# gevaertlab/sequoia-pub

Hardware: AMD Instinct MI355X
Metric: slides/sec (1000-patch WSI, UNI-dim, 20k-gene head) (higher is better)
Workload: dtype f16x3; 1 GPU; pipeline: 1000 x 224x224 uint8 patches/slide -> ResNet-50 embed -> k-Means(100) -> ViS(D=2048, depth 6, 16 heads, G=20820) forward (BASELINE config 3), patches uploaded from pinned host memory every step; embedder=ResNet-50 (src/resnet.py forward_extract), feature_dim=2048, patch_size=224, parallelism=slide-sharded x1

## Files before the change

### sequoia-pub_amd/csrc/conv1_x3.hip

```cpp
#include "gemm.h"
#include "x3_fmt.h"

namespace {

constexpr int TP = 8;
constexpr int TC = 2 * TP + 1;
constexpr int RW = 40;
constexpr int RH = 2 * TC + 5;
constexpr int IN_BYTES = RH * RW * 8;
constexpr int MT = 10;
constexpr int CROW = 272;
constexpr int COUT_BYTES = MT * 32 * CROW;
constexpr int LUT_BYTES = 2 * 3 * 256 * 2;
constexpr int W_LD = 152;
constexpr int NT = 512;
constexpr int RW_BYTES = 16384;
constexpr int LDS_BYTES = 2 * IN_BYTES + COUT_BYTES + LUT_BYTES + RW_BYTES;

struct Conv1X3Args {
    const uint8_t* u8;
    const float* f32;
    const uint16_t* w;
    long long w_plane;
    const float* bias;
    const float* colscale;
    uint16_t* out;
    long long out_plane;
    int n, H, W, tiles_y, tiles_x, tiles;
    const uint16_t* w1;
    int w1_tiled;
    const float* b1; const float* cs1;
    uint16_t* t1;
};

template <bool F16>
__global__ __launch_bounds__(NT) void conv1_pool_x3_kernel(const Conv1X3Args p) {
    using F = X3Fmt<F16>;
    extern __shared__ __attribute__((aligned(16))) char smem[];
    char* s_hi = smem;
    char* s_lo = smem + IN_BYTES;
    char* s_out = smem + 2 * IN_BYTES;
    uint16_t* s_lut = reinterpret_cast<uint16_t*>(smem + 2 * IN_BYTES + COUT_BYTES);
    const int tid = threadIdx.x, lane = tid & 63;
    const int wave = __builtin_amdgcn_readfirstlane(tid >> 6);
    const int wm = wave >> 1, wn = wave & 1;
    const int l31 = lane & 31, g = lane >> 5;
    const int tile0 = wm < 2 ? wm * 3 : 6 + (wm - 2) * 2;
    const int ntile = wm < 2 ? 3 : 2;

    for (int i = tid; i < 3 * 256; i += NT) {
        const int c = i >> 8, v = i & 255;
        const float mean = c == 0 ? 0.485f : (c == 1 ? 0.456f : 0.406f), sd = c == 0 ? 0.229f : (c == 1 ? 0.224f : 0.225f);
        const float x = ((float)v / 255.0f - mean) / sd;
        const uint32_t h = F::pack2(x, 0.f);
        const uint32_t l = F::pack2(x - F::lo_f(h), 0.f);
        s_lut[i] = (uint16_t)h;
        s_lut[768 + i] = (uint16_t)l;
    }

    u32x4 wh[14], wl[14];
    {
        const uint16_t* wr = p.w + (size_t)(wn * 32 + l31) * W_LD;
#pragma unroll
        for (int t = 0; t < 14; ++t) {
            const int ky = t >> 1, h = t & 1;
            union { u32x4 v; uint16_t u[8]; } fh, fl;
#pragma unroll
            for (int e = 0; e < 8; ++e) {
                const int kx = 4 * h + 2 * g + (e >> 2), c = e & 3;
                const bool ok = kx < 7 && c < 3;
                const int k = ok ? (ky * 7 + kx) * 3 + c : 0;
                fh.u[e] = ok ? wr[k] : (uint16_t)0;
                fl.u[e] = ok ? wr[p.w_plane + k] : (uint16_t)0;
            }
            wh[t] = fh.v; wl[t] = fl.v;
        }
    }
    const float bias = p.bias[wn * 32 + l31];
    const float cscale = p.colscale ? p.colscale[wn * 32 + l31] : 1.0f;
    const bool fuse = p.t1 != nullptr;
    const int ri = (wave >> 1) & 1, rj = wave & 1;
    char* const s_rw = smem + 2 * IN_BYTES + COUT_BYTES + LUT_BYTES;
    if (fuse) {
        for (int sl = tid; sl < 1024; sl += NT) {
            const int ln = sl & 63, pl = (sl >> 6) & 1, ks = (sl >> 7) & 3, j = sl >> 9;
            const int n = j * 32 + (ln & 31), k = ks * 16 + (ln >> 5) * 8;
            const size_t o = p.w1_tiled ? ((size_t)(k >> 5) * 64 + n) * 32 + (k & 31) : (size_t)n * 64 + k;
            *reinterpret_cast<u32x4*>(s_rw + sl * 16) = *reinterpret_cast<const u32x4*>(p.w1 + (pl ? p.w_plane : 0) + o);
        }
    }
    __syncthreads();

    int a_off[3];
#pragma unroll
    for (int i = 0; i < 3; ++i) {
        int m = (tile0 + i) * 32 + l31;
        if (m >= TC * TC) m = 0;
        const int oy = m / TC, ox = m - oy * TC;
        a_off[i] = ((2 * oy) * RW + 2 * ox + 2 * g) * 8;
    }

    const int H = p.H, W = p.W;
    const int OHc = (H + 1) / 2, OWc = (W + 1) / 2;
    const int PH = (OHc + 1) / 2, PW = (OWc + 1) / 2;
    const int tps2 = p.tiles_y * p.tiles_x;
    constexpr int NPX = (RH * RW + NT - 1) / NT;

    uint32_t pre01[NPX], pre2[NPX];
    uint32_t pre_ok = 0;
    auto prefetch = [&](int tile) {
        const int img = tile / tps2, tt = tile - img * tps2;
        const int ty = tt / p.tiles_x, tx = tt - ty * p.tiles_x;
        const int iy0 = 4 * TP * ty - 5, ix0 = 4 * TP * tx - 5;
        const uint8_t* base = p.u8 + (size_t)img * H * W * 3;
        pre_ok = 0;
#pragma unroll
        for (int j = 0; j < NPX; ++j) {
            const int idx = tid + j * NT;
            const int r = idx / RW, q = idx - r * RW;
            const int iy = iy0 + r, ix = ix0 + q;
            const bool ok = idx < RH * RW && (unsigned)iy < (unsigned)H && (unsigned)ix < (unsigned)W;
            const uint8_t* px = base + ((uint32_t)(ok ? iy : 0) * W + (ok ? ix : 0)) * 3;
            uint16_t v01;
            __builtin_memcpy(&v01, px, 2);
            pre01[j] = v01; pre2[j] = px[2];
            pre_ok |= ok ? (1u << j) : 0u;
        }
    };
    auto commit = [&]() {
#pragma unroll
        for (int j = 0; j < NPX; ++j) {
            const int idx = tid + j * NT;
            if (idx < RH * RW) {
                const bool ok = (pre_ok >> j) & 1;
                const uint32_t c0 = pre01[j] & 0xffu, c1 = (pre01[j] >> 8) & 0xffu, c2 = pre2[j] & 0xffu;
                const uint32_t h01 = ok ? ((uint32_t)s_lut[c0] | ((uint32_t)s_lut[256 + c1] << 16)) : 0u;
                const uint32_t h2 = ok ? (uint32_t)s_lut[512 + c2] : 0u;
                const uint32_t l01 = ok ? ((uint32_t)s_lut[768 + c0] | ((uint32_t)s_lut[768 + 256 + c1] << 16)) : 0u;
                const uint32_t l2 = ok ? (uint32_t)s_lut[768 + 512 + c2] : 0u;
                *reinterpret_cast<u32x2*>(s_hi + idx * 8) = u32x2{h01, h2};
                *reinterpret_cast<u32x2*>(s_lo + idx * 8) = u32x2{l01, l2};
            }
        }
    };
    if (p.u8 && (int)blockIdx.x < p.tiles) prefetch(blockIdx.x);

    for (int tile = blockIdx.x; tile < p.tiles; tile += gridDim.x) {
        const int img = tile / tps2;
        const int tt = tile - img * tps2;
        const int ty = tt / p.tiles_x, tx = tt - ty * p.tiles_x;

        if (p.u8) {
            commit();
        } else {
            const int iy0 = 4 * TP * ty - 5, ix0 = 4 * TP * tx - 5;
            for (int idx = tid; idx < RH * RW; idx += NT) {
                const int r = idx / RW, q = idx - r * RW;
                const int iy = iy0 + r, ix = ix0 + q;
                u32x2 hv = {0, 0}, lv = {0, 0};
                if ((unsigned)iy < (unsigned)H && (unsigned)ix < (unsigned)W) {
                    const float* px = p.f32 + ((size_t)img * 3 * H + iy) * W + ix;
                    const float x0 = px[0], x1 = px[(size_t)H * W], x2 = px[2 * (size_t)H * W];
                    hv[0] = F::pack2(x0, x1); hv[1] = F::pack2(x2, 0.f);
                    lv[0] = F::rest2(x0, x1, hv[0]); lv[1] = F::pack2(x2 - F::lo_f(hv[1]), 0.f);
                }
                *reinterpret_cast<u32x2*>(s_hi + idx * 8) = hv;
                *reinterpret_cast<u32x2*>(s_lo + idx * 8) = lv;
            }
        }
        __syncthreads();
        if (p.u8 && tile + (int)gridDim.x < p.tiles) prefetch(tile + gridDim.x);

        f32x16 acc[3];
#pragma unroll
        for (int i = 0; i < 3; ++i)
#pragma unroll
            for (int r = 0; r < 16; ++r) acc[i][r] = 0.f;
#pragma unroll
        for (int t = 0; t < 14; ++t) {
            const int ky = t >> 1, h = t & 1;
            u32x4 ah[3], al[3];
#pragma unroll
            for (int i = 0; i < 3; ++i)
                if (i < ntile) {
                    ah[i] = *reinterpret_cast<const u32x4*>(s_hi + a_off[i] + (ky * RW + 4 * h) * 8);
                    al[i] = *reinterpret_cast<const u32x4*>(s_lo + a_off[i] + (ky * RW + 4 * h) * 8);
                }
#pragma unroll
            for (int i = 0; i < 3; ++i) if (i < ntile) F::mma(al[i], wh[t], acc[i]);
#pragma unroll
            for (int i = 0; i < 3; ++i) if (i < ntile) F::mma(ah[i], wl[t], acc[i]);
#pragma unroll
            for (int i = 0; i < 3; ++i) if (i < ntile) F::mma(ah[i], wh[t], acc[i]);
        }
        {
            char* dst = s_out + (tile0 * 32 + 4 * g) * CROW + (wn * 32 + l31) * 4;
#pragma unroll
            for (int i = 0; i < 3; ++i)
                if (i < ntile) {
#pragma unroll
                    for (int r = 0; r < 16; ++r) {
                        const int m0 = i * 32 + (r & 3) + 8 * (r >> 2);
                        *reinterpret_cast<float*>(dst + m0 * CROW) = fmaxf(cscale * acc[i][r] + bias, 0.f);
                    }
                }
        }
        __syncthreads();

        {
            const int pp = tid >> 3, cg = tid & 7;
            const int py = pp >> 3, px = pp & 7;
            float best[8];
#pragma unroll
            for (int e = 0; e < 8; ++e) best[e] = 0.f;
#pragma unroll
            for (int dy = 0; dy < 3; ++dy)
#pragma unroll
                for (int dx = 0; dx < 3; ++dx) {
                    int cy = 2 * py + dy, cx = 2 * px + dx;
                    if (ty == 0 && cy == 0) cy = 1;
                    if (tx == 0 && cx == 0) cx = 1;
                    if (2 * TP * ty + cy - 1 == OHc) cy -= 1;
                    if (2 * TP * tx + cx - 1 == OWc) cx -= 1;
                    const char* src = s_out + (cy * TC + cx) * CROW + cg * 32;
                    const f32x4 v0 = *reinterpret_cast<const f32x4*>(src), v1 = *reinterpret_cast<const f32x4*>(src + 16);
#pragma unroll
                    for (int e = 0; e < 4; ++e) { best[e] = fmaxf(best[e], v0[e]); best[4 + e] = fmaxf(best[4 + e], v1[e]); }
                }
            u32x4 hi, lo;
            x3_split8<F16>(best, hi, lo);
            if (TP * ty + py < PH && TP * tx + px < PW) {
                uint16_t* dst = p.out + (((size_t)img * PH + TP * ty + py) * PW + TP * tx + px) * 64 + cg * 8;
                *reinterpret_cast<u32x4*>(dst) = hi;
                *reinterpret_cast<u32x4*>(dst + p.out_plane) = lo;
            }
            if (fuse) {
                char* a = smem + pp * 128 + ((cg ^ ((pp >> 1) & 7)) << 4);
                *reinterpret_cast<u32x4*>(a) = hi;
                *reinterpret_cast<u32x4*>(a + 8192) = lo;
            }
        }
        if (fuse) {
            __syncthreads();
            if (wave < 4) {
                f32x16 racc;
#pragma unroll
                for (int r = 0; r < 16; ++r) racc[r] = 0.f;
                const int row = ri * 32 + l31;
                const char* arow = smem + row * 128;
                const int sw = (row >> 1) & 7;
#pragma unroll
                for (int ks = 0; ks < 4; ++ks) {
                    const u32x4 ah = *reinterpret_cast<const u32x4*>(arow + (((2 * ks + g) ^ sw) << 4));
                    const u32x4 al = *reinterpret_cast<const u32x4*>(arow + 8192 + (((2 * ks + g) ^ sw) << 4));
                    const u32x4 bh = *reinterpret_cast<const u32x4*>(s_rw + (((rj * 4 + ks) * 2) * 64 + lane) * 16);
                    const u32x4 bl = *reinterpret_cast<const u32x4*>(s_rw + (((rj * 4 + ks) * 2 + 1) * 64 + lane) * 16);
                    F::mma(al, bh, racc);
                    F::mma(ah, bl, racc);
                    F::mma(ah, bh, racc);
                }
                char* dst = s_out + (ri * 32 + 4 * g) * CROW + (rj * 32 + l31) * 4;
#pragma unroll
                for (int r = 0; r < 16; ++r) *reinterpret_cast<float*>(dst + ((r & 3) + 8 * (r >> 2)) * CROW) = racc[r];
            }
            __syncthreads();
            {
                const int pp = tid >> 3, cg = tid & 7;
                const int py = pp >> 3, px = pp & 7;
                const char* src = s_out + pp * CROW + cg * 32;
                const f32x4 a0 = *reinterpret_cast<const f32x4*>(src), a1 = *reinterpret_cast<const f32x4*>(src + 16);
                float v[8] = {a0[0], a0[1], a0[2], a0[3], a1[0], a1[1], a1[2], a1[3]};
                const f32x4 b0 = *reinterpret_cast<const f32x4*>(p.b1 + cg * 8), b1v = *reinterpret_cast<const f32x4*>(p.b1 + cg * 8 + 4);
                float sc[8] = {1.f, 1.f, 1.f, 1.f, 1.f, 1.f, 1.f, 1.f};
                if (p.cs1) {
                    const f32x4 s0 = *reinterpret_cast<const f32x4*>(p.cs1 + cg * 8), s1 = *reinterpret_cast<const f32x4*>(p.cs1 + cg * 8 + 4);
#pragma unroll
                    for (int e = 0; e < 4; ++e) { sc[e] = s0[e]; sc[4 + e] = s1[e]; }
                }
                const float bb[8] = {b0[0], b0[1], b0[2], b0[3], b1v[0], b1v[1], b1v[2], b1v[3]};
#pragma unroll
                for (int e = 0; e < 8; ++e) v[e] = x3_relu(sc[e] * v[e] + bb[e]);
                u32x4 hi, lo;
                x3_split8<F16>(v, hi, lo);
                if (TP * ty + py < PH && TP * tx + px < PW) {
                    uint16_t* dst = p.t1 + (((size_t)img * PH + TP * ty + py) * PW + TP * tx + px) * 64 + cg * 8;
                    *reinterpret_cast<u32x4*>(dst) = hi;
                    *reinterpret_cast<u32x4*>(dst + p.out_plane) = lo;
                }
            }
        }
    }
}

}

int sq_launch_conv1_pool_x3(int f16, const uint8_t* u8, const float* f32_nchw, const uint16_t* w152_hi, long long w_plane, const float* bias,
                            const float* colscale, uint16_t* out_hi, long long out_plane, int n, int H, int W, hipStream_t stream,
                            const uint16_t* w1_hi, int w1_tiled, const float* b1, const float* cs1, uint16_t* t1_hi) {
    SQ_REQUIRE(H >= 7 && W >= 7 && n >= 1, "conv1_pool_x3: n=%d patches of %d x %d", n, H, W);
    Conv1X3Args a;
    a.u8 = u8; a.f32 = f32_nchw; a.w = w152_hi; a.w_plane = w_plane; a.bias = bias; a.colscale = colscale;
    a.out = out_hi; a.out_plane = out_plane; a.n = n; a.H = H; a.W = W;
    SQ_REQUIRE(!t1_hi || (w1_hi && b1), "conv1_pool_x3: the fused reduce needs its weights and bias");
    a.w1 = w1_hi; a.w1_tiled = w1_tiled; a.b1 = b1; a.cs1 = cs1; a.t1 = t1_hi;
    const int PH = ((H + 1) / 2 + 1) / 2, PW = ((W + 1) / 2 + 1) / 2;
    a.tiles_y = (PH + TP - 1) / TP; a.tiles_x = (PW + TP - 1) / TP;
    const long long tiles = (long long)n * a.tiles_y * a.tiles_x;
    SQ_REQUIRE(tiles < (1ll << 31), "conv1_pool_x3: too many tiles");
    a.tiles = (int)tiles;
    static SqDevOnce attr;
    if (attr.needed()) {
        SQ_HIP_CHECK(hipFuncSetAttribute((const void*)conv1_pool_x3_kernel<false>, hipFuncAttributeMaxDynamicSharedMemorySize, LDS_BYTES));
        SQ_HIP_CHECK(hipFuncSetAttribute((const void*)conv1_pool_x3_kernel<true>, hipFuncAttributeMaxDynamicSharedMemorySize, LDS_BYTES));
        attr.done();
    }
    const int grid = (int)(tiles < 256 ? tiles : 256);
    int prof = -1;
    if (sq_prof_on()) {
        const double px_out = (double)n * ((H + 1) / 2) * ((W + 1) / 2);
        prof = sq_prof_begin(f16 ? (t1_hi ? "conv1_pool_reduce_f16x3" : "conv1_pool_f16x3") : (t1_hi ? "conv1_pool_reduce_bf16x3" : "conv1_pool_bf16x3"),
                             2.0 * px_out * 64 * 147 + (t1_hi ? 2.0 * n * PH * PW * 64.0 * 64.0 : 0.0),
                             (double)n * H * W * 3 + (double)n * PH * PW * 64 * 4 * (t1_hi ? 2 : 1), stream);
    }
    if (f16) hipLaunchKernelGGL(conv1_pool_x3_kernel<true>, dim3(grid), dim3(NT), LDS_BYTES, stream, a);
    else hipLaunchKernelGGL(conv1_pool_x3_kernel<false>, dim3(grid), dim3(NT), LDS_BYTES, stream, a);
    SQ_LAUNCH_CHECK();
    if (prof >= 0) sq_prof_end(prof, stream);
    return SQ_OK;
}
```

Before: 34.54 slides/s.

## Double-buffer conv1 input windows with space-to-depth layout and interleaved staging

Reorganizes the conv1 stem's shared-memory input window into a 2x2 space-to-depth cell layout, so the 7x7 stride-2 kernel needs 12 MMA k-steps instead of 14. The input window is double-buffered: the next tile's pixels are staged into the alternate buffer partway through the current tile's MMA loop, and the global prefetch runs two tiles ahead. The normalization LUT packs hi/lo into one word, and the reduce bias/scale moves into LDS. Debug bit flags that can disable stages are also added. The cost is more LDS and more complex indexing.

```diff
diff --git a/sequoia-pub_amd/csrc/conv1_x3.hip b/sequoia-pub_amd/csrc/conv1_x3.hip
--- a/sequoia-pub_amd/csrc/conv1_x3.hip
+++ b/sequoia-pub_amd/csrc/conv1_x3.hip
@@ -1,21 +1,32 @@
 #include "gemm.h"
 #include "x3_fmt.h"
 
+extern int g_dbg;
+
 namespace {
 
 constexpr int TP = 8;
 constexpr int TC = 2 * TP + 1;
-constexpr int RW = 40;
-constexpr int RH = 2 * TC + 5;
-constexpr int IN_BYTES = RH * RW * 8;
+constexpr int RH = 2 * TC + 6;
+constexpr int NCELL = RH / 2;
+constexpr int CELL = 24;
+constexpr int RP = 664;
+constexpr int NPAIR = RH * NCELL;
+constexpr int IN_BYTES = NCELL * RP;
+constexpr int SET_BYTES = 2 * IN_BYTES;
+constexpr int KS = 12;
 constexpr int MT = 10;
 constexpr int CROW = 272;
 constexpr int COUT_BYTES = MT * 32 * CROW;
-constexpr int LUT_BYTES = 2 * 3 * 256 * 2;
+constexpr int LUT_BYTES = 3 * 256 * 4;
 constexpr int W_LD = 152;
 constexpr int NT = 512;
 constexpr int RW_BYTES = 16384;
-constexpr int LDS_BYTES = 2 * IN_BYTES + COUT_BYTES + LUT_BYTES + RW_BYTES;
+constexpr int RB_BYTES = 2 * 64 * 4;
+constexpr int LDS_BYTES = 2 * SET_BYTES + COUT_BYTES + LUT_BYTES + RW_BYTES + RB_BYTES;
+static_assert(SET_BYTES >= 16384 && SET_BYTES % 16 == 0, "the reduce's A image lives in the current tile's window planes");
+static_assert(LDS_BYTES <= 160 * 1024, "LDS");
+typedef uint32_t u32x2a8 __attribute__((ext_vector_type(2), aligned(8)));
 
 struct Conv1X3Args {
     const uint8_t* u8;
@@ -31,16 +42,15 @@
     int w1_tiled;
     const float* b1; const float* cs1;
     uint16_t* t1;
+    int dbg;
 };
 
 template <bool F16>
 __global__ __launch_bounds__(NT) void conv1_pool_x3_kernel(const Conv1X3Args p) {
     using F = X3Fmt<F16>;
     extern __shared__ __attribute__((aligned(16))) char smem[];
-    char* s_hi = smem;
-    char* s_lo = smem + IN_BYTES;
-    char* s_out = smem + 2 * IN_BYTES;
-    uint16_t* s_lut = reinterpret_cast<uint16_t*>(smem + 2 * IN_BYTES + COUT_BYTES);
+    char* s_out = smem + 2 * SET_BYTES;
+    uint32_t* s_lut = reinterpret_cast<uint32_t*>(smem + 2 * SET_BYTES + COUT_BYTES);
     const int tid = threadIdx.x, lane = tid & 63;
     const int wave = __builtin_amdgcn_readfirstlane(tid >> 6);
     const int wm = wave >> 1, wn = wave & 1;
@@ -54,21 +64,23 @@
         const float x = ((float)v / 255.0f - mean) / sd;
         const uint32_t h = F::pack2(x, 0.f);
         const uint32_t l = F::pack2(x - F::lo_f(h), 0.f);
-        s_lut[i] = (uint16_t)h;
-        s_lut[768 + i] = (uint16_t)l;
-    }
-
-    u32x4 wh[14], wl[14];
+        s_lut[i] = (h & 0xffffu) | (l << 16);
+    }
+
+    u32x4 wh[KS], wl[KS];
     {
         const uint16_t* wr = p.w + (size_t)(wn * 32 + l31) * W_LD;
 #pragma unroll
-        for (int t = 0; t < 14; ++t) {
-            const int ky = t >> 1, h = t & 1;
+        for (int t = 0; t < KS; ++t) {
+            const int kyc = t / 3, s = t - 3 * kyc;
             union { u32x4 v; uint16_t u[8]; } fh, fl;
 #pragma unroll
             for (int e = 0; e < 8; ++e) {
-                const int kx = 4 * h + 2 * g + (e >> 2), c = e & 3;
-                const bool ok = kx < 7 && c < 3;
+                const int j = s * 16 + g * 8 + e;
+                const int kxc = j / 12, r = j - 12 * kxc;
+                const int dy = r / 6, dx = (r / 3) & 1, c = r % 3;
+                const int ky = 2 * kyc + dy, kx = 2 * kxc + dx;
+                const bool ok = ky < 7 && kx < 7;
                 const int k = ok ? (ky * 7 + kx) * 3 + c : 0;
                 fh.u[e] = ok ? wr[k] : (uint16_t)0;
                 fl.u[e] = ok ? wr[p.w_plane + k] : (uint16_t)0;
@@ -80,8 +92,10 @@
     const float cscale = p.colscale ? p.colscale[wn * 32 + l31] : 1.0f;
     const bool fuse = p.t1 != nullptr;
     const int ri = (wave >> 1) & 1, rj = wave & 1;
-    char* const s_rw = smem + 2 * IN_BYTES + COUT_BYTES + LUT_BYTES;
+    char* const s_rw = smem + 2 * SET_BYTES + COUT_BYTES + LUT_BYTES;
+    float* const s_rb = reinterpret_cast<float*>(s_rw + RW_BYTES);
     if (fuse) {
+        if (tid < 64) { s_rb[tid] = p.b1[tid]; s_rb[64 + tid] = p.cs1 ? p.cs1[tid] : 1.f; }
         for (int sl = tid; sl < 1024; sl += NT) {
             const int ln = sl & 63, pl = (sl >> 6) & 1, ks = (sl >> 7) & 3, j = sl >> 9;
             const int n = j * 32 + (ln & 31), k = ks * 16 + (ln >> 5) * 8;
@@ -91,22 +105,25 @@
     }
     __syncthreads();
 
-    int a_off[3];
+    int a_off[3], a_off8[3];
 #pragma unroll
     for (int i = 0; i < 3; ++i) {
         int m = (tile0 + i) * 32 + l31;
         if (m >= TC * TC) m = 0;
         const int oy = m / TC, ox = m - oy * TC;
-        a_off[i] = ((2 * oy) * RW + 2 * ox + 2 * g) * 8;
+        a_off[i] = oy * RP + ox * CELL + g * 16;
+        a_off8[i] = a_off[i] + 8;
+        asm volatile("" : "+v"(a_off8[i]));
     }
 
     const int H = p.H, W = p.W;
     const int OHc = (H + 1) / 2, OWc = (W + 1) / 2;
     const int PH = (OHc + 1) / 2, PW = (OWc + 1) / 2;
     const int tps2 = p.tiles_y * p.tiles_x;
-    constexpr int NPX = (RH * RW + NT - 1) / NT;
-
-    uint32_t pre01[NPX], pre2[NPX];
+    constexpr int NPR = (NPAIR + NT - 1) / NT;
+
+    auto pair_off = [&](int idx) { const int r = idx / NCELL, C = idx - r * NCELL; return (r >> 1) * RP + C * CELL + (r & 1) * 12; };
+    uint32_t pre01[2 * NPR], pre2[2 * NPR];
     uint32_t pre_ok = 0;
     auto prefetch = [&](int tile) {
         const int img = tile / tps2, tt = tile - img * tps2;
@@ -115,11 +132,11 @@
         const uint8_t* base = p.u8 + (size_t)img * H * W * 3;
         pre_ok = 0;
 #pragma unroll
-        for (int j = 0; j < NPX; ++j) {
-            const int idx = tid + j * NT;
-            const int r = idx / RW, q = idx - r * RW;
+        for (int j = 0; j < 2 * NPR; ++j) {
+            const int idx = tid + (j >> 1) * NT;
+            const int r = idx / NCELL, q = 2 * (idx - r * NCELL) + (j & 1);
             const int iy = iy0 + r, ix = ix0 + q;
-            const bool ok = idx < RH * RW && (unsigned)iy < (unsigned)H && (unsigned)ix < (unsigned)W;
+            const bool ok = idx < NPAIR && r < RH - 1 && q < RH - 1 && (unsigned)iy < (unsigned)H && (unsigned)ix < (unsigned)W;
             const uint8_t* px = base + ((uint32_t)(ok ? iy : 0) * W + (ok ? ix : 0)) * 3;
             uint16_t v01;
             __builtin_memcpy(&v01, px, 2);
@@ -127,72 +144,109 @@
             pre_ok |= ok ? (1u << j) : 0u;
         }
     };
-    auto commit = [&]() {
-#pragma unroll
-        for (int j = 0; j < NPX; ++j) {
-            const int idx = tid + j * NT;
-            if (idx < RH * RW) {
+    auto commit = [&](int jr, char* set) {
+        const int idx = tid + jr * NT;
+        if (idx < NPAIR) {
+            uint32_t e[6];
+#pragma unroll
+            for (int q = 0; q < 2; ++q) {
+                const int j = 2 * jr + q;
                 const bool ok = (pre_ok >> j) & 1;
                 const uint32_t c0 = pre01[j] & 0xffu, c1 = (pre01[j] >> 8) & 0xffu, c2 = pre2[j] & 0xffu;
-                const uint32_t h01 = ok ? ((uint32_t)s_lut[c0] | ((uint32_t)s_lut[256 + c1] << 16)) : 0u;
-                const uint32_t h2 = ok ? (uint32_t)s_lut[512 + c2] : 0u;
-                const uint32_t l01 = ok ? ((uint32_t)s_lut[768 + c0] | ((uint32_t)s_lut[768 + 256 + c1] << 16)) : 0u;
-                const uint32_t l2 = ok ? (uint32_t)s_lut[768 + 512 + c2] : 0u;
-                *reinterpret_cast<u32x2*>(s_hi + idx * 8) = u32x2{h01, h2};
-                *reinterpret_cast<u32x2*>(s_lo + idx * 8) = u32x2{l01, l2};
+                e[3 * q] = ok ? s_lut[c0] : 0u;
+                e[3 * q + 1] = ok ? s_lut[256 + c1] : 0u;
+                e[3 * q + 2] = ok ? s_lut[512 + c2] : 0u;
+            }
+            uint32_t* dh = reinterpret_cast<uint32_t*>(set + pair_off(idx));
+            uint32_t* dl = reinterpret_cast<uint32_t*>(set + IN_BYTES + pair_off(idx));
+#pragma unroll
+            for (int w = 0; w < 3; ++w) {
+                dh[w] = (e[2 * w] & 0xffffu) | (e[2 * w + 1] << 16);
+                dl[w] = (e[2 * w] >> 16) | (e[2 * w + 1] & 0xffff0000u);
             }
         }
     };
-    if (p.u8 && (int)blockIdx.x < p.tiles) prefetch(blockIdx.x);
-
-    for (int tile = blockIdx.x; tile < p.tiles; tile += gridDim.x) {
+    auto stage_f32 = [&](int tile, int jr, char* set) {
+        const int img = tile / tps2, tt = tile - img * tps2;
+        const int ty = tt / p.tiles_x, tx = tt - ty * p.tiles_x;
+        const int iy0 = 4 * TP * ty - 5, ix0 = 4 * TP * tx - 5;
+        const int idx = tid + jr * NT;
+        if (idx < NPAIR) {
+            const int r = idx / NCELL, q0 = 2 * (idx - r * NCELL);
+            float x[6] = {0.f, 0.f, 0.f, 0.f, 0.f, 0.f};
+#pragma unroll
+            for (int q = 0; q < 2; ++q) {
+                const int iy = iy0 + r, ix = ix0 + q0 + q;
+                if (r < RH - 1 && q0 + q < RH - 1 && (unsigned)iy < (unsigned)H && (unsigned)ix < (unsigned)W) {
+                    const float* px = p.f32 + ((size_t)img * 3 * H + iy) * W + ix;
+                    x[3 * q] = px[0]; x[3 * q + 1] = px[(size_t)H * W]; x[3 * q + 2] = px[2 * (size_t)H * W];
+                }
+            }
+            uint32_t* dh = reinterpret_cast<uint32_t*>(set + pair_off(idx));
+            uint32_t* dl = reinterpret_cast<uint32_t*>(set + IN_BYTES + pair_off(idx));
+#pragma unroll
+            for (int w = 0; w < 3; ++w) {
+                const uint32_t h = F::pack2(x[2 * w], x[2 * w + 1]);
+                dh[w] = h;
+                dl[w] = F::rest2(x[2 * w], x[2 * w + 1], h);
+            }
+        }
+    };
+    const bool stage_on = !(p.dbg & 2);
+    auto stage = [&](int tile, int jr, char* set) {
+        if (!stage_on) return;
+        if (p.u8) commit(jr, set); else stage_f32(tile, jr, set);
+    };
+
+    const int G = gridDim.x;
+    if ((int)blockIdx.x < p.tiles) {
+        if (p.u8) prefetch(blockIdx.x);
+#pragma unroll
+        for (int jr = 0; jr < NPR; ++jr) stage(blockIdx.x, jr, smem);
+        if (p.u8 && (int)blockIdx.x + G < p.tiles) prefetch(blockIdx.x + G);
+    }
+    __syncthreads();
+
+    int cur = 0;
+    for (int tile = blockIdx.x; tile < p.tiles; tile += G, cur ^= 1) {
         const int img = tile / tps2;
         const int tt = tile - img * tps2;
         const int ty = tt / p.tiles_x, tx = tt - ty * p.tiles_x;
-
-        if (p.u8) {
-            commit();
-        } else {
-            const int iy0 = 4 * TP * ty - 5, ix0 = 4 * TP * tx - 5;
-            for (int idx = tid; idx < RH * RW; idx += NT) {
-                const int r = idx / RW, q = idx - r * RW;
-                const int iy = iy0 + r, ix = ix0 + q;
-                u32x2 hv = {0, 0}, lv = {0, 0};
-                if ((unsigned)iy < (unsigned)H && (unsigned)ix < (unsigned)W) {
-                    const float* px = p.f32 + ((size_t)img * 3 * H + iy) * W + ix;
-                    const float x0 = px[0], x1 = px[(size_t)H * W], x2 = px[2 * (size_t)H * W];
-                    hv[0] = F::pack2(x0, x1); hv[1] = F::pack2(x2, 0.f);
-                    lv[0] = F::rest2(x0, x1, hv[0]); lv[1] = F::pack2(x2 - F::lo_f(hv[1]), 0.f);
-                }
-                *reinterpret_cast<u32x2*>(s_hi + idx * 8) = hv;
-                *reinterpret_cast<u32x2*>(s_lo + idx * 8) = lv;
+        char* const s_hi = smem + cur * SET_BYTES;
+        char* const s_lo = s_hi + IN_BYTES;
+        char* const s_nxt = smem + (cur ^ 1) * SET_BYTES;
+        const bool more = tile + G < p.tiles;
+
+        f32x16 acc[3];
+#pragma unroll
+        for (int i = 0; i < 3; ++i)
+#pragma unroll
+            for (int r = 0; r < 16; ++r) acc[i][r] = 0.f;
+        const bool mma_on = !(p.dbg & 4);
+#pragma unroll
+        for (int t = 0; t < KS; ++t) {
+            if (t == 1 && more) stage(tile + G, 0, s_nxt);
+            if (t == 6 && more) stage(tile + G, 1, s_nxt);
+            if (mma_on) {
+                const int koff = (t / 3) * RP + (t % 3) * 32;
+                u32x4 ah[3], al[3];
+#pragma unroll
+                for (int i = 0; i < 3; ++i)
+                    if (i < ntile) {
+                        const u32x2a8 h0 = *reinterpret_cast<const u32x2a8*>(s_hi + a_off[i] + koff), h1 = *reinterpret_cast<const u32x2a8*>(s_hi + a_off8[i] + koff);
+                        const u32x2a8 l0 = *reinterpret_cast<const u32x2a8*>(s_lo + a_off[i] + koff), l1 = *reinterpret_cast<const u32x2a8*>(s_lo + a_off8[i] + koff);
+                        ah[i] = u32x4{h0[0], h0[1], h1[0], h1[1]};
+                        al[i] = u32x4{l0[0], l0[1], l1[0], l1[1]};
+                    }
+#pragma unroll
+                for (int i = 0; i < 3; ++i) if (i < ntile) F::mma(al[i], wh[t], acc[i]);
+#pragma unroll
+                for (int i = 0; i < 3; ++i) if (i < ntile) F::mma(ah[i], wl[t], acc[i]);
+#pragma unroll
+                for (int i = 0; i < 3; ++i) if (i < ntile) F::mma(ah[i], wh[t], acc[i]);
             }
         }
         __syncthreads();
-        if (p.u8 && tile + (int)gridDim.x < p.tiles) prefetch(tile + gridDim.x);
-
-        f32x16 acc[3];
-#pragma unroll
-        for (int i = 0; i < 3; ++i)
-#pragma unroll
-            for (int r = 0; r < 16; ++r) acc[i][r] = 0.f;
-#pragma unroll
-        for (int t = 0; t < 14; ++t) {
-            const int ky = t >> 1, h = t & 1;
-            u32x4 ah[3], al[3];
-#pragma unroll
-            for (int i = 0; i < 3; ++i)
-                if (i < ntile) {
-                    ah[i] = *reinterpret_cast<const u32x4*>(s_hi + a_off[i] + (ky * RW + 4 * h) * 8);
-                    al[i] = *reinterpret_cast<const u32x4*>(s_lo + a_off[i] + (ky * RW + 4 * h) * 8);
-                }
-#pragma unroll
-            for (int i = 0; i < 3; ++i) if (i < ntile) F::mma(al[i], wh[t], acc[i]);
-#pragma unroll
-            for (int i = 0; i < 3; ++i) if (i < ntile) F::mma(ah[i], wl[t], acc[i]);
-#pragma unroll
-            for (int i = 0; i < 3; ++i) if (i < ntile) F::mma(ah[i], wh[t], acc[i]);
-        }
         {
             char* dst = s_out + (tile0 * 32 + 4 * g) * CROW + (wn * 32 + l31) * 4;
 #pragma unroll
@@ -206,6 +260,7 @@
                 }
         }
         __syncthreads();
+        if (p.u8 && tile + 2 * G < p.tiles) prefetch(tile + 2 * G);
 
         {
             const int pp = tid >> 3, cg = tid & 7;
@@ -213,6 +268,7 @@
             float best[8];
 #pragma unroll
             for (int e = 0; e < 8; ++e) best[e] = 0.f;
+            if (!(p.dbg & 8))
 #pragma unroll
             for (int dy = 0; dy < 3; ++dy)
 #pragma unroll
@@ -229,25 +285,25 @@
                 }
             u32x4 hi, lo;
             x3_split8<F16>(best, hi, lo);
-            if (TP * ty + py < PH && TP * tx + px < PW) {
+            if (TP * ty + py < PH && TP * tx + px < PW && !(p.dbg & 1)) {
                 uint16_t* dst = p.out + (((size_t)img * PH + TP * ty + py) * PW + TP * tx + px) * 64 + cg * 8;
                 *reinterpret_cast<u32x4*>(dst) = hi;
                 *reinterpret_cast<u32x4*>(dst + p.out_plane) = lo;
             }
             if (fuse) {
-                char* a = smem + pp * 128 + ((cg ^ ((pp >> 1) & 7)) << 4);
+                char* a = s_hi + pp * 128 + ((cg ^ ((pp >> 1) & 7)) << 4);
                 *reinterpret_cast<u32x4*>(a) = hi;
                 *reinterpret_cast<u32x4*>(a + 8192) = lo;
             }
         }
         if (fuse) {
             __syncthreads();
-            if (wave < 4) {
+            if (wave < 4 && !(p.dbg & 16)) {
                 f32x16 racc;
 #pragma unroll
                 for (int r = 0; r < 16; ++r) racc[r] = 0.f;
                 const int row = ri * 32 + l31;
-                const char* arow = smem + row * 128;
+                const char* arow = s_hi + row * 128;
                 const int sw = (row >> 1) & 7;
 #pragma unroll
                 for (int ks = 0; ks < 4; ++ks) {
@@ -270,19 +326,15 @@
                 const char* src = s_out + pp * CROW + cg * 32;
                 const f32x4 a0 = *reinterpret_cast<const f32x4*>(src), a1 = *reinterpret_cast<const f32x4*>(src + 16);
                 float v[8] = {a0[0], a0[1], a0[2], a0[3], a1[0], a1[1], a1[2], a1[3]};
-                const f32x4 b0 = *reinterpret_cast<const f32x4*>(p.b1 + cg * 8), b1v = *reinterpret_cast<const f32x4*>(p.b1 + cg * 8 + 4);
-                float sc[8] = {1.f, 1.f, 1.f, 1.f, 1.f, 1.f, 1.f, 1.f};
-                if (p.cs1) {
-                    const f32x4 s0 = *reinterpret_cast<const f32x4*>(p.cs1 + cg * 8), s1 = *reinterpret_cast<const f32x4*>(p.cs1 + cg * 8 + 4);
-#pragma unroll
-                    for (int e = 0; e < 4; ++e) { sc[e] = s0[e]; sc[4 + e] = s1[e]; }
-                }
+                const f32x4 b0 = *reinterpret_cast<const f32x4*>(s_rb + cg * 8), b1v = *reinterpret_cast<const f32x4*>(s_rb + cg * 8 + 4);
+                const f32x4 s0 = *reinterpret_cast<const f32x4*>(s_rb + 64 + cg * 8), s1 = *reinterpret_cast<const f32x4*>(s_rb + 64 + cg * 8 + 4);
+                const float sc[8] = {s0[0], s0[1], s0[2], s0[3], s1[0], s1[1], s1[2], s1[3]};
                 const float bb[8] = {b0[0], b0[1], b0[2], b0[3], b1v[0], b1v[1], b1v[2], b1v[3]};
 #pragma unroll
                 for (int e = 0; e < 8; ++e) v[e] = x3_relu(sc[e] * v[e] + bb[e]);
                 u32x4 hi, lo;
                 x3_split8<F16>(v, hi, lo);
-                if (TP * ty + py < PH && TP * tx + px < PW) {
+                if (TP * ty + py < PH && TP * tx + px < PW && !(p.dbg & 1)) {
                     uint16_t* dst = p.t1 + (((size_t)img * PH + TP * ty + py) * PW + TP * tx + px) * 64 + cg * 8;
                     *reinterpret_cast<u32x4*>(dst) = hi;
                     *reinterpret_cast<u32x4*>(dst + p.out_plane) = lo;
@@ -302,7 +354,7 @@
     a.u8 = u8; a.f32 = f32_nchw; a.w = w152_hi; a.w_plane = w_plane; a.bias = bias; a.colscale = colscale;
     a.out = out_hi; a.out_plane = out_plane; a.n = n; a.H = H; a.W = W;
     SQ_REQUIRE(!t1_hi || (w1_hi && b1), "conv1_pool_x3: the fused reduce needs its weights and bias");
-    a.w1 = w1_hi; a.w1_tiled = w1_tiled; a.b1 = b1; a.cs1 = cs1; a.t1 = t1_hi;
+    a.w1 = w1_hi; a.w1_tiled = w1_tiled; a.b1 = b1; a.cs1 = cs1; a.t1 = t1_hi; a.dbg = g_dbg;
     const int PH = ((H + 1) / 2 + 1) / 2, PW = ((W + 1) / 2 + 1) / 2;
     a.tiles_y = (PH + TP - 1) / TP; a.tiles_x = (PW + TP - 1) / TP;
     const long long tiles = (long long)n * a.tiles_y * a.tiles_x;
@@ -328,3 +380,16 @@
     if (prof >= 0) sq_prof_end(prof, stream);
     return SQ_OK;
 }
+
+extern "C" int sq_dbg_conv1_pool_x3(int f16, const void* u8, const float* f32_nchw, const void* w_hi, const void* w_lo, const float* bias,
+                                    const float* colscale, const void* w1_hi, const void* w1_lo, const float* b1, const float* cs1,
+                                    int w1_tiled, void* out_hi, void* out_lo, void* t1_hi, void* t1_lo, int n, int H, int W, void* stream) {
+    const uint16_t* w = (const uint16_t*)w_hi;
+    uint16_t* out = (uint16_t*)out_hi; uint16_t* t1 = (uint16_t*)t1_hi;
+    const long long plW = (const uint16_t*)w_lo - w, plO = (uint16_t*)out_lo - out;
+    SQ_REQUIRE((u8 != nullptr) != (f32_nchw != nullptr), "dbg_conv1_pool_x3: exactly one input form");
+    SQ_REQUIRE(!t1 || ((const uint16_t*)w1_lo - (const uint16_t*)w1_hi == plW && (uint16_t*)t1_lo - t1 == plO),
+               "dbg_conv1_pool_x3: the reduce's weights and output must share the stem's plane distances");
+    return sq_launch_conv1_pool_x3(f16, (const uint8_t*)u8, f32_nchw, w, plW, bias, colscale, out, plO, n, H, W, (hipStream_t)stream,
+                                   (const uint16_t*)w1_hi, w1_tiled, b1, cs1, t1);
+}
```

New measurement: 34.69 slides/s (median of 6 runs). Within noise of the previous version (+0.4%).
